# mikael-jorda/sai2-primitives-perso

Measured on AMD Instinct MI355X. Metric: control-ticks/sec (node), 65k batched 7-DOF Panda, 2-task hierarchy, higher is better.
Workload: dtype f64

## Files before the change

### sai2-primitives-perso_amd/csrc/sai2b_fast.hpp

```cpp
#pragma once
#include "sai2b_device.hpp"

namespace sai2b {

template <int n, class Mat>
DI void chol(const Mat& A, real* L, real* dinv) {
	UNROLL for (int j = 0; j < n; j++) {
		real s = A[j * n + j];
		UNROLL for (int k = 0; k < j; k++) s = fma(-L[j * n + k], L[j * n + k], s);
		real r = rsqrt(s);
		dinv[j] = r;
		L[j * n + j] = s * r;
		UNROLL for (int i = j + 1; i < n; i++) {
			real t = A[i * n + j];
			UNROLL for (int k = 0; k < j; k++) t = fma(-L[i * n + k], L[j * n + k], t);
			L[i * n + j] = t * r;
		}
	}
}
template <int n>
DI void solve_lower(const real* L, const real* dinv, real* x) {
	UNROLL for (int i = 0; i < n; i++) {
		real t = x[i];
		UNROLL for (int k = 0; k < i; k++) t = fma(-L[i * n + k], x[k], t);
		x[i] = t * dinv[i];
	}
}
template <int n>
DI void solve_lower_t(const real* L, const real* dinv, real* x) {
	UNROLL for (int i = n - 1; i >= 0; i--) {
		real t = x[i];
		UNROLL for (int k = i + 1; k < n; k++) t = fma(-L[k * n + i], x[k], t);
		x[i] = t * dinv[i];
	}
}

DI bool certify_nonsingular(const real* J, real s_abs_tol, real s_max) {
	real G[36];
	mm_nt_sym<6, N>(J, J, G);
	return certify_gram<6>(G, nullptr, s_abs_tol * s_abs_tol, s_max * s_max);
}

struct JtEarly {
	real f[N], ddq[N], integ[N];
};
template <class Rows>
DI void fast_jt_early(const DevTask& t1, const RobotCtx& rc, const Rows& r, JtEarly& e) {
	UNROLL for (int i = 0; i < N; i++) {
		const real qd = r.law_goal(i), dqd = r.law_goal(N + i);
		e.ddq[i] = r.law_goal(2 * N + i);
		const real integ = fma(rc.q[i] - qd, t1.dt, r.state(i));
		e.integ[i] = integ;
		if (t1.use_vsat) {
			const real kvi = gain_pinv(t1.kv[i]);
			real dv = -t1.kp[i] * kvi * (rc.q[i] - qd) - t1.ki[i] * kvi * integ;
			dv = fmin(fmax(dv, -t1.vsat[i]), t1.vsat[i]);
			e.f[i] = -t1.kv[i] * (rc.dq[i] - dv);
		} else {
			e.f[i] = -t1.kp[i] * (rc.q[i] - qd) - t1.kv[i] * (rc.dq[i] - dqd) - t1.ki[i] * integ;
		}
	}
}

#define SAI2B_PHASE() do { __builtin_amdgcn_sched_barrier(0); asm volatile("; SAI2B_PHASE_MARK"); __builtin_amdgcn_sched_barrier(0); } while (0)
#if defined(__HIP_DEVICE_COMPILE__)
#define SAI2B_CHAIN_PHASE() SAI2B_PHASE()
#endif
}
#include "sai2b_chain.h"
namespace sai2b {

template <int FAST, bool PAY = false>
struct StageLayout {
	static constexpr bool JT_STAGED = FAST == 2 && PAY, PARKED = FAST == 2 && !PAY;
	static constexpr int DQ = 0, JG = N, JS = JG + (JT_STAGED ? 3 * N : 0), MG = JS + (JT_STAGED ? N : 0);
	static constexpr int MS = MG + 24, PLD = MS + 6, ROWS = PLD + (PAY ? PAYLOAD_ROWS : 0);
	static constexpr int PAIRS = (ROWS + 1) / 2;
	static constexpr int IROW = 2 * PAIRS;
	static constexpr int IMAGE = IROW * 64 + 32;
	static constexpr int MROWS = N * (N + 1) / 2;
	static constexpr int DOUBLES = IMAGE + (PARKED ? (MROWS + N) * 64 : 0);
};

template <int FAST, bool PAY = false>
DI const real* stage_row(const DevParams& P, int k) {
	using S = StageLayout<FAST, PAY>;
	const int B = P.B;
	if (k >= S::ROWS) k = S::ROWS - 1;
	if (k < S::JG) return P.dq + (size_t)(k - S::DQ) * B;
	if (k < S::JS) return P.task[1].law_goals + (size_t)(k - S::JG) * B;
	if (k < S::MG) return P.task[1].state + (size_t)(k - S::JS) * B;
	if (k < S::MS) return P.task[0].law_goals + (size_t)(k - S::MG) * B;
	if constexpr (PAY) {
		if (k >= S::PLD) return P.payload + (size_t)(k - S::PLD) * B;
	}
	return P.task[0].state + (size_t)(k - S::MS) * B;
}

DI void glds(const void* src, real* lds, int bytes) {
	typedef __attribute__((address_space(1))) void gvoid;
	typedef __attribute__((address_space(3))) void lvoid;
	if (bytes == 16)
		__builtin_amdgcn_global_load_lds((gvoid*)src, (lvoid*)lds, 16, 0, 0);
	else
		__builtin_amdgcn_global_load_lds((gvoid*)src, (lvoid*)lds, 4, 0, 0);
}

template <int FAST, bool PAY = false>
DI void stage_issue(const DevParams& P, real* img, int b0) {
	using S = StageLayout<FAST, PAY>;
	const int B = P.B, lane = threadIdx.x;
	if ((B & 1) == 0) {
		const int col = min(b0 + 2 * (lane & 31), B - 2);
		const bool hi = lane >= 32;
		UNROLL for (int i = 0; i < S::PAIRS; i++)
			glds((hi ? stage_row<FAST, PAY>(P, 2 * i + 1) : stage_row<FAST, PAY>(P, 2 * i)) + col, img + 2 * i * 64, 16);
	} else {
		UNROLL for (int h = 0; h < 2; h++) {
			const int col = min(b0 + 32 * h + (lane >> 1), B - 1);
			UNROLL for (int k = 0; k < S::ROWS; k++)
				glds((const int*)(stage_row<FAST, PAY>(P, k) + col) + (lane & 1), img + k * 64 + 32 * h, 4);
		}
	}
	glds(P.task[0].istate + (size_t)IS_NTYPES * B + min(b0 + lane, B - 1), img + S::IROW * 64, 4);
}

struct StagedRows {
	const DevTask& t;
	int B, b;
	const real* lg;
	const real* st;
	int st_rows;
	DI real law_goal(int k) const { return lg[k * 64]; }
	DI real goal(int k) const { return ld(t.goals, k, B, b); }
	DI real sensed(int k) const { return ld(t.sensed, k, B, b); }
	DI real state(int k) const { return k < st_rows ? st[k * 64] : ld(t.state, k, B, b); }
};

struct LdsSym {
	const real* col;
	DI real operator[](int k) const {
		const int i = k / N, j = k % N;
		return col[(i * (i + 1) / 2 + j) * 64];
	}
};

struct JtGiven {
	const JtEarly& e;
	DI void prefetch() {}
	DI void prefetch_q() {}
	DI void project(const real* a, real& af, real& aacc) {
		UNROLL for (int i = 0; i < N; i++) {
			af = fma(a[i], e.f[i], af);
			aacc = fma(a[i], e.ddq[i], aacc);
		}
	}
};
struct JtLate {
	const DevTask& t1;
	int B, b;
	const real* dq;
	const real* qrows;
	real lg[3 * N], s[N], q[N];
	struct Rows {
		const real *lg, *s;
		DI real law_goal(int k) const { return lg[k]; }
		DI real state(int k) const { return s[k]; }
	};
	DI void prefetch() {
		UNROLL for (int k = 0; k < 3 * N; k++) lg[k] = ld(t1.law_goals, k, B, b);
		UNROLL for (int i = 0; i < N; i++) s[i] = ld(t1.state, i, B, b);
	}
	DI void prefetch_q() {
		UNROLL for (int i = 0; i < N; i++) q[i] = ld(qrows, i, B, b);
	}
	DI void project(const real* a, real& af, real& aacc) {
		RobotCtx rc;
		UNROLL for (int i = 0; i < N; i++) {
			asm volatile("" : "+v"(q[i]) : "v"(a[0]));
			rc.q[i] = q[i];
			rc.dq[i] = dq[i * 64];
		}
		JtEarly e;
		fast_jt_early(t1, rc, Rows{lg, s}, e);
		UNROLL for (int i = 0; i < N; i++) st(t1.state, i, B, b, e.integ[i]);
		JtGiven{e}.project(a, af, aacc);
	}
};

template <class Mat>
DI void fast_tick_mft(const DevParams& P, const real* J, const Mat& M, const real* Fu, const real* Ff, real* tau) {
	const DevTask& t0 = P.task[0];

	const bool mft_bie = t0.decoupling == SAI2B_BOUNDED_INERTIA_ESTIMATES;
	const bool mft_full = t0.decoupling == SAI2B_FULL_DYNAMIC_DECOUPLING;
	const bool any_bie = mft_bie;
	const real thr = t0.bie_threshold;
	real LB[N * N], dB[N], z[6];
	UNROLL for (int i = 0; i < 6; i++) z[i] = Fu[i];
	if (any_bie) {
		real MB[N * N];
		UNROLL for (int i = 0; i < N; i++) UNROLL for (int j = 0; j <= i; j++) MB[i * N + j] = M[i * N + j];
		UNROLL for (int i = 0; i < N; i++) MB[i * N + i] = fmax(MB[i * N + i], thr);
		chol<N>(MB, LB, dB);
	}
	if (mft_bie) {
		real YB[N * 6], AB[36], LAB[36], dAB[6];
		UNROLL for (int c = 0; c < 6; c++) {
			real colb[N];
			UNROLL for (int i = 0; i < N; i++) colb[i] = J[c * N + i];
			solve_lower<N>(LB, dB, colb);
			UNROLL for (int i = 0; i < N; i++) YB[i * 6 + c] = colb[i];
		}
		UNROLL for (int i = 0; i < 6; i++) UNROLL for (int j = 0; j <= i; j++) {
			real s = 0;
			UNROLL for (int l = 0; l < N; l++) s = fma(YB[l * 6 + i], YB[l * 6 + j], s);
			AB[i * 6 + j] = s;
			AB[j * 6 + i] = s;
		}
		chol<6>(AB, LAB, dAB);
		solve_lower<6>(LAB, dAB, z);
		solve_lower_t<6>(LAB, dAB, z);
	}
	SAI2B_PHASE();
	real L[N * N], dL[N], Y[N * 6];
	chol<N>(M, L, dL);
	UNROLL for (int c = 0; c < 6; c++) {
		real col[N];
		UNROLL for (int i = 0; i < N; i++) col[i] = J[c * N + i];
		solve_lower<N>(L, dL, col);
		UNROLL for (int i = 0; i < N; i++) Y[i * 6 + c] = col[i];
	}
	SAI2B_PHASE();
	if (mft_full) {
		real A[36], LA[36], dA[6];
		UNROLL for (int i = 0; i < 6; i++) UNROLL for (int j = 0; j <= i; j++) {
			real s = 0;
			UNROLL for (int l = 0; l < N; l++) s = fma(Y[l * 6 + i], Y[l * 6 + j], s);
			A[i * 6 + j] = s;
			A[j * 6 + i] = s;
		}
		chol<6>(A, LA, dA);
		solve_lower<6>(LA, dA, z);
		solve_lower_t<6>(LA, dA, z);
	}
	SAI2B_PHASE();
	UNROLL for (int i = 0; i < 6; i++) z[i] += Ff[i];
	real yz[N], tau_mft[N];
	mv<N, 6>(Y, z, yz);
	UNROLL for (int i = 0; i < N; i++) {
		real s = 0;
		UNROLL for (int k = 0; k <= i; k++) s = fma(L[i * N + k], yz[k], s);
		tau_mft[i] = s;
	}
	UNROLL for (int i = 0; i < N; i++) tau[i] = tau_mft[i];
}

template <bool HAS_JT, class Mat, class JT>
DI void fast_tick(const DevParams& P, const real* J, const Mat& M, const real* Fu, const real* Ff, int B, int b,
				  bool with_comp, JT& jt, real* tau) {
	if constexpr (!HAS_JT) {
		fast_tick_mft(P, J, M, Fu, Ff, tau);
	} else {
		const DevTask &t0 = P.task[0], &t1 = P.task[1];
		const bool jt_bie = t1.decoupling == SAI2B_BOUNDED_INERTIA_ESTIMATES;
		chain::tick2<N>(J, M, Fu, Ff, t0.decoupling == SAI2B_BOUNDED_INERTIA_ESTIMATES,
						t0.decoupling == SAI2B_FULL_DYNAMIC_DECOUPLING, t1.decoupling == SAI2B_FULL_DYNAMIC_DECOUPLING,
						t1.decoupling == SAI2B_IMPEDANCE, jt_bie ? t1.bie_threshold : t0.bie_threshold, with_comp, jt, tau);
	}
}

}
```

### sai2-primitives-perso_amd/csrc/sai2b_fast_body.hpp

```cpp
#pragma once
#include <hip/hip_runtime.h>

#include "sai2b_device.hpp"
#include "sai2b_fast.hpp"
#include "sai2b_baked_panda.h"
#include "sai2b_baked_panda_model.h"

namespace sai2b {

#if SAI2B_N == 7
DI void fk(const PandaBaked&, const real* q, Frames& F) {
	real sn[N], cs[N];
	UNROLL for (int i = 0; i < N; i++) sincos_joint(q[i], &sn[i], &cs[i]);
	panda_fk(sn, cs, F);
}
DI void jacobian(const PandaBaked&, const DevTask& t, const Frames& F, const real* x, real* J) { panda_jacobian(F, t.link, x, J); }
DI void mass_matrix(const PandaBaked&, const Frames& F, real* M, const NoPayload& = NoPayload{}) { panda_mass_matrix(F, M); }
DI void mass_matrix(const PandaBaked&, const Frames& F, real* M, const Payload& pl) {
	PayloadTerms pt;
	payload_terms(pl, F, pt);
	panda_mass_matrix_payload(F, pl.link, pt, M);
}
DI void gravity_vector(const PandaBaked&, const Frames& F, real* g, const NoPayload& = NoPayload{}) { panda_gravity_vector(F, g); }
DI void gravity_vector(const PandaBaked&, const Frames& F, real* g, const Payload& pl) {
	PayloadTerms pt;
	payload_terms(pl, F, pt);
	panda_gravity_vector_payload(F, pl.link, pt, g);
}

template <bool BAKED, class PL>
DI void fast_model(const DevParams& P, const Frames& F, const PL& pl, real* M, real* g) {
	if constexpr (BAKED)
		mass_matrix(PandaBaked{}, F, M, pl);
	else
		mass_matrix(P.model, F, M, pl);
	if (P.gravity_comp) {
		if constexpr (BAKED)
			gravity_vector(PandaBaked{}, F, g, pl);
		else
			gravity_vector(P.model, F, g, pl);
	}
	else {
		UNROLL for (int i = 0; i < N; i++) g[i] = 0;
	}
}

template <bool SELF>
DI bool fast_declined(int* __restrict__ fb_counts, int* __restrict__ fb_list, int parity, bool mine, int b) {
	if constexpr (SELF)
		return !mine;
	else
		return worklist_append(fb_counts, fb_list, parity, mine, b, fb_counts + 4);
}

template <bool BAKED, class PL, bool SELF = false>
DI bool tick_fast1_loads(const DevParams& P, int with_comp, int* __restrict__ fb_counts, int* __restrict__ fb_list, int parity,
						 int b) {
	const int B = P.B;
	RobotCtx rc;
	UNROLL for (int i = 0; i < N; i++) {
		rc.q[i] = ld(P.q, i, B, b);
		rc.dq[i] = ld(P.dq, i, B, b);
	}
	const DevTask& t0 = P.task[0];
	const bool clean = ldi(t0.istate, IS_NTYPES, B, b) == 0;
	JtEarly jt;
	MftIn in0;
	mft_load(t0, B, b, in0);
	SAI2B_PHASE();
	real J[6 * N], M[N * N], g[N], Fu[6], Ff[6];
	{
		Frames F;
		if constexpr (BAKED)
			fk(PandaBaked{}, rc.q, F);
		else
			fk(P.model, rc.q, F);
		real x[3], R[9];
		frame_pose(t0, F, x, R);
		if constexpr (BAKED)
			jacobian(PandaBaked{}, t0, F, x, J);
		else
			jacobian(P.model, t0, F, x, J);
		SAI2B_PHASE();
		mft_law(t0, rc, J, x, R, in0, Fu, Ff);
		SAI2B_PHASE();
		if constexpr (PL::on) {
			PL pl;
			payload_load(P.payload, P.payload_link, B, b, pl);
			fast_model<BAKED>(P, F, pl, M, g);
		} else {
			if constexpr (BAKED)
				mass_matrix(PandaBaked{}, F, M);
			else
				mass_matrix(P.model, F, M);
			if (P.gravity_comp) {
				if constexpr (BAKED)
					gravity_vector(PandaBaked{}, F, g);
				else
					gravity_vector(P.model, F, g);
			}
			else {
				UNROLL for (int i = 0; i < N; i++) g[i] = 0;
			}
		}
	}
	SAI2B_PHASE();
	const bool ok = certify_nonsingular(J, t0.s_abs_tol, t0.s_max);
	const bool mine = ok && clean;
	if (fast_declined<SELF>(fb_counts, fb_list, parity, mine, b)) return true;
	mft_store_integrators(t0, B, b, in0);
	SAI2B_PHASE();
	real tau[N];
	JtGiven none{jt};
	fast_tick<false>(P, J, M, Fu, Ff, B, b, with_comp != 0, none, tau);
	UNROLL for (int i = 0; i < N; i++) st(P.tau, i, B, b, tau[i] + g[i]);
	return false;
}

template <int FAST, bool BAKED, class PL, bool SELF = false>
DI bool tick_fast_body(const DevParams* __restrict__ Pp, int with_comp, int* __restrict__ fb_counts, int* __restrict__ fb_list,
					   int parity, real* img) {
	const DevParams& P = *Pp;
	const int B = P.B;
	const int b0 = blockIdx.x * 64, b = b0 + threadIdx.x;
	using S = StageLayout<FAST, PL::on>;
	RobotCtx rc;
	UNROLL for (int i = 0; i < N; i++) {
		rc.q[i] = ld(P.q, i, B, min(b, B - 1));
		asm volatile("" : "+v"(rc.q[i]));
	}
	SAI2B_PHASE();
	stage_issue<FAST, PL::on>(P, img, b0);
	SAI2B_PHASE();
	if (b >= B) return false;
	const DevTask& t0 = P.task[0];
	const real* col = img + threadIdx.x;
	real J[6 * N], x[3], R[9];
	{
		Frames F;
		if constexpr (BAKED)
			fk(PandaBaked{}, rc.q, F);
		else
			fk(P.model, rc.q, F);
		frame_pose(t0, F, x, R);
		if constexpr (BAKED)
			jacobian(PandaBaked{}, t0, F, x, J);
		else
			jacobian(P.model, t0, F, x, J);
		if constexpr (S::PARKED) {
			SAI2B_PHASE();
			real M[N * N], g[N];
			fast_model<BAKED>(P, F, PL{}, M, g);
			real* park = img + S::IMAGE + threadIdx.x;
			UNROLL for (int i = 0; i < N; i++) UNROLL for (int j = 0; j <= i; j++) park[(i * (i + 1) / 2 + j) * 64] = M[i * N + j];
			UNROLL for (int i = 0; i < N; i++) park[(S::MROWS + i) * 64] = g[i];
		}
	}
	SAI2B_PHASE();
	const bool ok = certify_nonsingular(J, t0.s_abs_tol, t0.s_max);
	SAI2B_PHASE();
	__syncthreads();
	UNROLL for (int i = 0; i < N; i++) {
		rc.dq[i] = col[(S::DQ + i) * 64];
		if constexpr (!S::PARKED) rc.q[i] = ld(P.q, i, B, b);
	}
	const bool clean = ((const int*)(img + S::IROW * 64))[threadIdx.x] == 0;
	MftIn in0;
	mft_load(t0, StagedRows{t0, B, b, col + S::MG * 64, col + S::MS * 64, 6}, in0);
	SAI2B_PHASE();
	real Fu[6], Ff[6];
	mft_law(t0, rc, J, x, R, in0, Fu, Ff);
	SAI2B_PHASE();
	real tau[N];
	if constexpr (S::PARKED) {
		const bool mine = ok && clean;
		if (fast_declined<SELF>(fb_counts, fb_list, parity, mine, b)) return true;
		mft_store_integrators(t0, B, b, in0);
		SAI2B_PHASE();
		const real* park = col + S::IMAGE;
		JtLate jt{P.task[1], B, b, col + S::DQ * 64, P.q};
		fast_tick<FAST == 2>(P, J, LdsSym{park}, Fu, Ff, B, b, with_comp != 0, jt, tau);
		UNROLL for (int i = 0; i < N; i++) st(P.tau, i, B, b, tau[i] + park[(S::MROWS + i) * 64]);
	} else {
		real M[N * N], g[N];
		{
			PL pl;
			if constexpr (PL::on) {
				pl.link = P.payload_link;
				pl.m = col[S::PLD * 64];
				UNROLL for (int k = 0; k < 3; k++) pl.c[k] = col[(S::PLD + 1 + k) * 64];
				UNROLL for (int k = 0; k < 6; k++) pl.I[k] = col[(S::PLD + 4 + k) * 64];
			}
			Frames F;
			if constexpr (BAKED)
				fk(PandaBaked{}, rc.q, F);
			else
				fk(P.model, rc.q, F);
			fast_model<BAKED>(P, F, pl, M, g);
		}
		SAI2B_PHASE();
		const bool mine = ok && clean;
		if (fast_declined<SELF>(fb_counts, fb_list, parity, mine, b)) return true;
		JtEarly e;
		if constexpr (FAST == 2) fast_jt_early(P.task[1], rc, StagedRows{P.task[1], B, b, col + S::JG * 64, col + S::JS * 64, N}, e);
		mft_store_integrators(t0, B, b, in0);
		if (FAST == 2) {
			UNROLL for (int i = 0; i < N; i++) st(P.task[1].state, i, B, b, e.integ[i]);
		}
		SAI2B_PHASE();
		JtGiven jt{e};
		fast_tick<FAST == 2>(P, J, M, Fu, Ff, B, b, with_comp != 0, jt, tau);
		UNROLL for (int i = 0; i < N; i++) st(P.tau, i, B, b, tau[i] + g[i]);
	}
	return false;
}
#endif

}
```

### sai2-primitives-perso_amd/csrc/sai2b_host.cpp

```cpp
#include <hip/hip_runtime.h>

#include <algorithm>
#include <cmath>
#include <cstdio>
#include <cstdlib>
#include <chrono>
#include <cstring>
#include <string>
#include <vector>

#include "sai2b_launch.h"
#include "sai2b_snapshot_layout.h"
#include "sai2b_reset_sampler_layout.h"
#include "sai2b_env_sampler_layout.h"
#include "sai2b_model_host.h"
#include "sai2b_baked_panda.h"

using sai2b::DevModel;
using sai2b::rot_from_rpy;
using sai2b::sym3_from6;
using sai2b::DevParams;
using sai2b::DevTask;
using sai2b::TickCall;
using sai2b::TickForm;
using sai2b::WorkList;
constexpr int N = SAI2B_N;

static thread_local std::string g_error;

extern "C" void sai2b_shared_error_set(const char* msg);

struct sai2b_ctx {
	int dof_tag = N;
	int B = 0, T = 0, device = 0;
	bool introspection = false;
	bool models_fresh = false;
	bool params_dirty = true;
	bool baked_model = false;
	bool blocking_sync = false;
	sai2b::RouteSwitches sw;
	sai2b::TickRoute route;
	WorkList fb, rg, otg, tk;
	int* fb_seen = nullptr;
	hipEvent_t fb_seen_ev = nullptr;
	unsigned long long* fb_report = nullptr;
	bool update_pending = false;
	double* q_pose = nullptr;
	bool q_is_pose = true;
	unsigned goals_dirty = ~0u;
	bool otg_all_idle = false, no_otg_idle_skip = false;
	unsigned long long goals_epoch = 0, otg_obs_epoch = 0;
	int* otg_busy_seen = nullptr;
	hipEvent_t otg_seen_ev = nullptr;
	sai2b::DelayedLook otg_look;
	bool goals_exposed = false;
	sai2b_robot_model model;
	sai2b_task_config cfg[SAI2B_MAX_TASKS];
	DevParams h_params;
	DevParams* d_params = nullptr;
	hipStream_t stream = nullptr;
	hipStream_t caller_stream = nullptr;
	hipEvent_t ev_in = nullptr, ev_out = nullptr;
	double *q = nullptr, *dq = nullptr, *tau = nullptr;
	double* status_buf = nullptr;
// ... 552 lines not shown
	d.otg_jerk = (c.use_internal_otg && c.internal_otg_jerk_limited) ? 1 : 0;
	d.otg_n = c.type == SAI2B_JOINT_TASK ? c.task_dof : 6;
	for (int i = 0; i < sai2b::OTG_MD; i++) {
		if (c.type == SAI2B_JOINT_TASK) {
			d.otg_vmax[i] = i < c.task_dof ? c.otg_max_velocity[i] : 0.0;
			d.otg_amax[i] = i < c.task_dof ? c.otg_max_acceleration[i] : 0.0;
			d.otg_jmax[i] = i < c.task_dof ? c.otg_max_jerk[i] : 0.0;
		} else {
			d.otg_vmax[i] = i < 3 ? c.otg_max_linear_velocity : i < 6 ? c.otg_max_angular_velocity : 0.0;
			d.otg_amax[i] = i < 3 ? c.otg_max_linear_acceleration : i < 6 ? c.otg_max_angular_acceleration : 0.0;
			d.otg_jmax[i] = i < 3 ? c.otg_max_linear_jerk : i < 6 ? c.otg_max_angular_jerk : 0.0;
		}
	}
}

template <class T>
static int dev_alloc(sai2b_ctx* ctx, T** p, size_t count) {
	void* v = nullptr;
	HIP_TRY(ctx, hipMalloc(&v, std::max<size_t>(count, 1) * sizeof(T)));
	HIP_TRY(ctx, hipMemsetAsync(v, 0, std::max<size_t>(count, 1) * sizeof(T), ctx->stream));
	ctx->allocs.push_back(v);
	*p = (T*)v;
	return SAI2B_OK;
}

static int popc_reinit(sai2b_ctx* ctx, int task) {
	DevTask& d = ctx->h_params.task[task];
	const size_t B = ctx->B;
	int rc;
	if (!d.popc_f) {
		if ((rc = dev_alloc(ctx, &d.popc_f, 4 * B))) return rc;
		if ((rc = dev_alloc(ctx, &d.popc_i, 3 * B))) return rc;
		if ((rc = dev_alloc(ctx, &d.popc_q, (size_t)sai2b::POPC_RING * B))) return rc;
		ctx->params_dirty = true;
	}
	std::vector<double> f(4 * B, 0.0);
	std::fill(f.begin() + 3 * B, f.end(), 1.0);
	std::vector<int> iv(3 * B, 0);
	std::fill(iv.begin(), iv.begin() + B, sai2b::POPC_MAX_COUNTER);
	HIP_TRY(ctx, hipMemcpyAsync(d.popc_f, f.data(), f.size() * sizeof(double), hipMemcpyHostToDevice, ctx->stream));
	HIP_TRY(ctx, hipMemcpyAsync(d.popc_i, iv.data(), iv.size() * sizeof(int), hipMemcpyHostToDevice, ctx->stream));
	HIP_TRY(ctx, hipStreamSynchronize(ctx->stream));
	return SAI2B_OK;
}

static int upload_params(sai2b_ctx* ctx) {
	if (!ctx->params_dirty) return SAI2B_OK;
	ctx->h_params.any_bie = 0, ctx->h_params.bie_thr = 0;
	for (int t = 0; t < ctx->h_params.n_tasks; t++)
		if (ctx->h_params.task[t].decoupling == SAI2B_BOUNDED_INERTIA_ESTIMATES) {
			ctx->h_params.any_bie = 1;
			ctx->h_params.bie_thr = ctx->h_params.task[t].bie_threshold;
		}
	HIP_TRY(ctx, hipMemcpyAsync(ctx->d_params, &ctx->h_params, sizeof(DevParams), hipMemcpyHostToDevice, ctx->stream));
	DevParams meas;
	if (ctx->js_on) {
		meas = ctx->h_params;
		meas.q = ctx->js_qm, meas.dq = ctx->js_dqm;
		HIP_TRY(ctx, hipMemcpyAsync(ctx->d_params_meas, &meas, sizeof(DevParams), hipMemcpyHostToDevice, ctx->stream));
	}
	HIP_TRY(ctx, hipStreamSynchronize(ctx->stream));
	ctx->params_dirty = false;
	return SAI2B_OK;
}

static int create_impl(sai2b_ctx* ctx, const sai2b_robot_model* model, const sai2b_task_config* tasks, int n_tasks,
					   int batch, int device) {
	int ndev = 0;
	if (hipGetDeviceCount(&ndev) != hipSuccess || ndev <= 0)
		return set_error(ctx, SAI2B_RUNTIME_ERROR, "sai2b_create: no HIP device available (this library has no CPU path)");
	if (device < 0 || device >= ndev) return set_error(ctx, SAI2B_INVALID_ARGUMENT, "sai2b_create: bad device index");
	HIP_TRY(ctx, hipSetDevice(device));
	HIP_TRY(ctx, hipStreamCreateWithFlags(&ctx->stream, hipStreamNonBlocking));
	HIP_TRY(ctx, hipEventCreateWithFlags(&ctx->ev_in, hipEventDisableTiming));
	HIP_TRY(ctx, hipEventCreateWithFlags(&ctx->ev_out, hipEventDisableTiming));
	ctx->B = batch, ctx->T = n_tasks, ctx->device = device;
	ctx->model = *model;
	ctx->sw = sai2b::route_switches_from_env();
	ctx->route = sai2b::TickRoute(ctx->sw);
	ctx->blocking_sync = sai2b::env_flag("SAI2B_BLOCKING_SYNC");
	ctx->no_otg_idle_skip = sai2b::env_flag("SAI2B_NO_OTG_IDLE_SKIP");
	DevParams& hp = ctx->h_params;
	std::memset(&hp, 0, sizeof(hp));
	hp.B = batch, hp.n_tasks = n_tasks;
	sai2b::host_fill_dev_model(*model, hp.model);
	if constexpr (N == 7) {
		using PB = sai2b::PandaBaked;
		const DevModel& m = hp.model;
		ctx->baked_model = std::memcmp(m.E, PB::E, sizeof(m.E)) == 0 && std::memcmp(m.xyz, PB::xyz, sizeof(m.xyz)) == 0 &&
						   std::memcmp(m.mass, PB::mass, sizeof(m.mass)) == 0 && std::memcmp(m.com, PB::com, sizeof(m.com)) == 0 &&
						   std::memcmp(m.inertia, PB::inertia, sizeof(m.inertia)) == 0 &&
						   std::memcmp(m.gravity, PB::gravity, sizeof(m.gravity)) == 0 &&
						   std::memcmp(m.jtype, PB::jtype, sizeof(m.jtype)) == 0;
		if (sai2b::env_flag("SAI2B_NO_BAKED_MODEL")) ctx->baked_model = false;
	}
	const size_t Bs = (size_t)batch;
	int rc;
	if ((rc = dev_alloc(ctx, &ctx->d_params, 1))) return rc;
	if ((rc = dev_alloc(ctx, &ctx->q, N * Bs))) return rc;
	if ((rc = dev_alloc(ctx, &ctx->dq, N * Bs))) return rc;
	if ((rc = dev_alloc(ctx, &ctx->tau, N * Bs))) return rc;
	hp.q = ctx->q, hp.dq = ctx->dq, hp.tau = ctx->tau;
	if ((rc = dev_alloc(ctx, &ctx->q_pose, (size_t)N * Bs))) return rc;
	if ((rc = dev_alloc(ctx, &ctx->fb.counts, 6))) return rc;
	HIP_TRY(ctx, hipHostMalloc((void**)&ctx->fb_report, 3 * sizeof(unsigned long long), hipHostMallocMapped | hipHostMallocCoherent));
	ctx->fb_report[0] = ctx->fb_report[1] = ctx->fb_report[2] = 0;
	HIP_TRY(ctx, hipHostGetDevicePointer((void**)&ctx->fb.report, ctx->fb_report, 0));
	if ((rc = dev_alloc(ctx, &ctx->fb.list, Bs))) return rc;
	if ((rc = dev_alloc(ctx, &ctx->rg.counts, 2))) return rc;
	if ((rc = dev_alloc(ctx, &ctx->rg.list, Bs))) return rc;
	HIP_TRY(ctx, hipHostMalloc((void**)&ctx->fb_seen, 2 * sizeof(int), hipHostMallocDefault));
// ... 3449 lines not shown
```

### sai2-primitives-perso_amd/csrc/sai2b_params.h

```cpp
#pragma once
#include "../../include/sai2b.h"

namespace sai2b {

#ifndef SAI2B_N
#define SAI2B_N 7
#endif
constexpr int N = SAI2B_N;
static_assert(N >= 1 && N <= SAI2B_MAX_DOF, "SAI2B_N");

struct DevModel {
	double E[N][9];
	double xyz[N][3];
	double mass[N];
	double com[N][3];
	double inertia[N][6];
	double q_lower[N], q_upper[N], effort[N];
	double gravity[3];
	int jtype[N];
};

constexpr int OTG_MD = N > 7 ? N : 7;

struct DevTask {
	int type;
	int decoupling;
	double bie_threshold;
	double dt;
	int k0;
	int full_selection;
	double S[N * N];
	double kp[N], kv[N], ki[N];
	int use_vsat;
	double vsat[N];
	int link;
	double frame_pos[3], frame_rot[9];
	int frame_rigid;
	int full_projection;
	int plain_motion;
	double P[36];
	double PU[36];
	int rank;
	int p_lead;
	int in_frame;
	double kp_pos[3], kv_pos[3], ki_pos[3], kp_ori[3], kv_ori[3], ki_ori[3];
	double kp_f[3], kv_f[3], ki_f[3], kp_m[3], kv_m[3], ki_m[3];
	double kff_f, kff_m, max_f, max_m;
	int cl_force, cl_moment, fdim, mdim;
	int passivity;
	double faxis[3], maxis[3];
	double sig[4][9];
	double lin_vsat, ang_vsat;
	double sensor_rot[9], sensor_pos[3];
// ... 20 lines not shown
	double* popc_f;
	int* popc_i;
	double* popc_q;
	double* dbg_tau;
	double* dbg_N;
	double* dbg_sigma;
	double* dbg_J;
	double* dbg_pose;
	double* dbg_F;
};

constexpr int MFT_GOAL_ROWS = 30;
constexpr int MFT_MOTION_GOAL_ROWS = 24;
constexpr int MFT_GOAL_POS = 0, MFT_GOAL_ROT = 3, MFT_GOAL_LIN_VEL = 12, MFT_GOAL_ANG_VEL = 15, MFT_GOAL_LIN_ACC = 18, MFT_GOAL_ANG_ACC = 21,
			  MFT_GOAL_FORCE = 24, MFT_GOAL_MOMENT = 27;
static_assert(MFT_GOAL_ANG_ACC + 3 == MFT_MOTION_GOAL_ROWS && MFT_MOTION_GOAL_ROWS == 24 && MFT_GOAL_FORCE == MFT_MOTION_GOAL_ROWS &&
				  MFT_GOAL_MOMENT + 3 == MFT_GOAL_ROWS && MFT_GOAL_ROWS == 30,
			  "goal rows of a MotionForceTask");
constexpr int OTG_IN = 0;
constexpr int OTG_CI = 5 * OTG_MD;
constexpr int OTG_OUT = 10 * OTG_MD;
constexpr int OTG_TIME = 13 * OTG_MD, OTG_DURATION = OTG_TIME + 1, OTG_GOAL_REACHED = OTG_TIME + 2, OTG_RESULT = OTG_TIME + 3,
			  OTG_TARGET_SET = OTG_TIME + 4, OTG_CI_INIT = OTG_TIME + 5, OTG_CI_EPOCH = OTG_TIME + 6, OTG_CONSTRUCTED = OTG_TIME + 7;
constexpr int OTG_TRAJ = OTG_TIME + 8;
constexpr int OTG_TRAJ_STRIDE = 13;
constexpr int OTG3_BRAKE = 0, OTG3_TSUM = 11, OTG3_J = 18, OTG3_A = 25, OTG3_V = 33, OTG3_P = 41, OTG3_STRIDE = 49;
constexpr int OTG_CART = OTG_TRAJ + OTG_MD * OTG_TRAJ_STRIDE;
constexpr int OTG_CART_REF = OTG_CART, OTG_CART_GOAL_R = OTG_CART + 9, OTG_CART_GOAL_W = OTG_CART + 18;
constexpr int OTG_IN_SYNC = OTG_CART + 21;
constexpr int OTG_ACTIVE = OTG_CART + 22;
constexpr int OTG_ROWS = OTG_CART + 23;
static_assert(N > 7 || (OTG_TRAJ == 99 && OTG_CART == 190 && OTG_IN_SYNC == 211), "row layout of the 7-DoF builds");
constexpr int MFT_QPRIOR = 12, MFT_DQPRIOR = 12 + N, MFT_T2DIR = 12 + 2 * N;
constexpr int MFT_STATE_ROWS = 12 + 3 * N;
constexpr int MFT_ISTATE_ROWS = 12;
constexpr int POPC_RING = 1024;
constexpr int POPC_WINDOW = 250, POPC_MAX_COUNTER = 50;
constexpr int IS_NTYPES = 7, IS_COUNT = 8, IS_SIZE = 9, IS_C1 = 10, IS_C2 = 11;

constexpr int PAYLOAD_ROWS = 10;
constexpr int CONTACT_ROWS = 9;
constexpr int CONTACT_STATUS_ROWS = 2 * SAI2B_MAX_CONTACT_POINTS + 6;

enum TickCertBits {
	TICK_CERT_COMP = 1,
	TICK_CERT_NO_INLANE = 2
};
enum TaskCertBits {
	TASK_CERT_TORQUE = 1,
	TASK_CERT_COMMIT = 2,
	TASK_CERT_NO_INLANE = 4
};

struct DevParams {
	int B;
	int n_tasks;
	int gravity_comp;
	int any_bie;
	const double* q;
	const double* dq;
	double* tau;
	double* dbg_M;
	double bie_thr;
	DevModel model;
	DevTask task[SAI2B_MAX_TASKS];
	const double* payload;
	const double* plant_payload;
	int payload_link, plant_payload_link;
	const double* contact;
	double* contact_status;
	int* contact_count;
	int contact_link, contact_n_points, contact_sensor_task, contact_reserved;
	double contact_points[SAI2B_MAX_CONTACT_POINTS][3];
	double contact_v_eps;
};

}
```

Baseline: 3.428 billion.

## Pack fast-path kernel parameters into cache-line-aligned block with scalar-register loads

Adds a FastBlock to DevParams, filled on the host, that groups the pointers, flags and gains used by the fast tick path into 64-byte-aligned groups. The kernel reads these grouped fields and pins them to scalar registers with inline-asm ties, replacing scattered loads from the large DevTask structs and runtime decoupling comparisons with a precomputed flags word. A specialised plain-motion law and a split Jt gain burst are also added. The aim is fewer, burstier scalar parameter loads and less register pressure, at the cost of duplicated parameter state that must stay in sync with the host fill.

```diff
diff --git a/sai2-primitives-perso_amd/csrc/sai2b_fast.hpp b/sai2-primitives-perso_amd/csrc/sai2b_fast.hpp
--- a/sai2-primitives-perso_amd/csrc/sai2b_fast.hpp
+++ b/sai2-primitives-perso_amd/csrc/sai2b_fast.hpp
@@ -44,22 +44,58 @@
 struct JtEarly {
 	real f[N], ddq[N], integ[N];
 };
+template <class T>
+DI void sgpr_tie(T& v) {
+	asm volatile("" : "+s"(v));
+}
+struct JtGains {
+	real dt, kp[N], kv[N], ki[N], vsat[N];
+};
+template <bool VSAT>
+DI void jt_gains_burst(const FastJt& s, JtGains& g) {
+	g.dt = s.dt;
+	UNROLL for (int i = 0; i < N; i++) {
+		g.kp[i] = s.kp[i], g.kv[i] = s.kv[i], g.ki[i] = s.ki[i];
+		if constexpr (VSAT) g.vsat[i] = s.vsat[i];
+	}
+	sgpr_tie(g.dt);
+	UNROLL for (int i = 0; i < N; i++) {
+		sgpr_tie(g.kp[i]), sgpr_tie(g.kv[i]), sgpr_tie(g.ki[i]);
+		if constexpr (VSAT) sgpr_tie(g.vsat[i]);
+	}
+}
 template <class Rows>
-DI void fast_jt_early(const DevTask& t1, const RobotCtx& rc, const Rows& r, JtEarly& e) {
-	UNROLL for (int i = 0; i < N; i++) {
-		const real qd = r.law_goal(i), dqd = r.law_goal(N + i);
-		e.ddq[i] = r.law_goal(2 * N + i);
-		const real integ = fma(rc.q[i] - qd, t1.dt, r.state(i));
-		e.integ[i] = integ;
-		if (t1.use_vsat) {
-			const real kvi = gain_pinv(t1.kv[i]);
-			real dv = -t1.kp[i] * kvi * (rc.q[i] - qd) - t1.ki[i] * kvi * integ;
-			dv = fmin(fmax(dv, -t1.vsat[i]), t1.vsat[i]);
-			e.f[i] = -t1.kv[i] * (rc.dq[i] - dv);
-		} else {
-			e.f[i] = -t1.kp[i] * (rc.q[i] - qd) - t1.kv[i] * (rc.dq[i] - dqd) - t1.ki[i] * integ;
-		}
-	}
+DI void fast_jt_law(const JtGains& g, bool use_vsat, const RobotCtx& rc, const Rows& r, JtEarly& e) {
+	if (use_vsat) {
+		UNROLL for (int i = 0; i < N; i++) {
+			const real qd = r.law_goal(i);
+			e.ddq[i] = r.law_goal(2 * N + i);
+			const real integ = fma(rc.q[i] - qd, g.dt, r.state(i));
+			e.integ[i] = integ;
+			const real kvi = gain_pinv(g.kv[i]);
+			real dv = -g.kp[i] * kvi * (rc.q[i] - qd) - g.ki[i] * kvi * integ;
+			dv = fmin(fmax(dv, -g.vsat[i]), g.vsat[i]);
+			e.f[i] = -g.kv[i] * (rc.dq[i] - dv);
+		}
+	} else {
+		UNROLL for (int i = 0; i < N; i++) {
+			const real qd = r.law_goal(i), dqd = r.law_goal(N + i);
+			e.ddq[i] = r.law_goal(2 * N + i);
+			const real integ = fma(rc.q[i] - qd, g.dt, r.state(i));
+			e.integ[i] = integ;
+			e.f[i] = -g.kp[i] * (rc.q[i] - qd) - g.kv[i] * (rc.dq[i] - dqd) - g.ki[i] * integ;
+		}
+	}
+}
+
+template <class Rows>
+DI void fast_jt_early(const FastJt& t1, bool use_vsat, const RobotCtx& rc, const Rows& r, JtEarly& e) {
+	JtGains g;
+	if (use_vsat)
+		jt_gains_burst<true>(t1, g);
+	else
+		jt_gains_burst<false>(t1, g);
+	fast_jt_law(g, use_vsat, rc, r, e);
 }
 
 #define SAI2B_PHASE() do { __builtin_amdgcn_sched_barrier(0); asm volatile("; SAI2B_PHASE_MARK"); __builtin_amdgcn_sched_barrier(0); } while (0)
@@ -83,18 +119,18 @@
 };
 
 template <int FAST, bool PAY = false>
-DI const real* stage_row(const DevParams& P, int k) {
+DI const real* stage_row(const FastEntry& P, int k) {
 	using S = StageLayout<FAST, PAY>;
 	const int B = P.B;
 	if (k >= S::ROWS) k = S::ROWS - 1;
 	if (k < S::JG) return P.dq + (size_t)(k - S::DQ) * B;
-	if (k < S::JS) return P.task[1].law_goals + (size_t)(k - S::JG) * B;
-	if (k < S::MG) return P.task[1].state + (size_t)(k - S::JS) * B;
-	if (k < S::MS) return P.task[0].law_goals + (size_t)(k - S::MG) * B;
+	if (k < S::JS) return P.law_goals1 + (size_t)(k - S::JG) * B;
+	if (k < S::MG) return P.state1 + (size_t)(k - S::JS) * B;
+	if (k < S::MS) return P.law_goals0 + (size_t)(k - S::MG) * B;
 	if constexpr (PAY) {
 		if (k >= S::PLD) return P.payload + (size_t)(k - S::PLD) * B;
 	}
-	return P.task[0].state + (size_t)(k - S::MS) * B;
+	return P.state0 + (size_t)(k - S::MS) * B;
 }
 
 DI void glds(const void* src, real* lds, int bytes) {
@@ -107,7 +143,7 @@
 }
 
 template <int FAST, bool PAY = false>
-DI void stage_issue(const DevParams& P, real* img, int b0) {
+DI void stage_issue(const FastEntry& P, real* img, int b0) {
 	using S = StageLayout<FAST, PAY>;
 	const int B = P.B, lane = threadIdx.x;
 	if ((B & 1) == 0) {
@@ -122,7 +158,7 @@
 				glds((const int*)(stage_row<FAST, PAY>(P, k) + col) + (lane & 1), img + k * 64 + 32 * h, 4);
 		}
 	}
-	glds(P.task[0].istate + (size_t)IS_NTYPES * B + min(b0 + lane, B - 1), img + S::IROW * 64, 4);
+	glds(P.istate0 + (size_t)IS_NTYPES * B + min(b0 + lane, B - 1), img + S::IROW * 64, 4);
 }
 
 struct StagedRows {
@@ -137,6 +173,83 @@
 	DI real state(int k) const { return k < st_rows ? st[k * 64] : ld(t.state, k, B, b); }
 };
 
+DI void frame_pose(const FastPose& t, const Frames& F, real* x, real* R) {
+	real Rl[9], pl[3];
+	UNROLL for (int k = 0; k < 9; k++) Rl[k] = F.R[N - 1][k];
+	UNROLL for (int k = 0; k < 3; k++) pl[k] = F.p[N - 1][k];
+	UNROLL for (int i = 0; i < N - 1; i++)
+		if (t.link == i) {
+			UNROLL for (int k = 0; k < 9; k++) Rl[k] = F.R[i][k];
+			UNROLL for (int k = 0; k < 3; k++) pl[k] = F.p[i][k];
+		}
+	UNROLL for (int k = 0; k < 3; k++)
+		x[k] = fma(Rl[3 * k], t.frame_pos[0], fma(Rl[3 * k + 1], t.frame_pos[1], fma(Rl[3 * k + 2], t.frame_pos[2], pl[k])));
+	mm<3, 3, 3>(Rl, t.frame_rot, R);
+}
+template <class MD>
+DI void jacobian(const MD& md, const FastPose& t, const Frames& F, const real* x, real* J) {
+	UNROLL for (int i = 0; i < N; i++) {
+		real z[3] = {F.R[i][2], F.R[i][5], F.R[i][8]};
+		real d[3] = {x[0] - F.p[i][0], x[1] - F.p[i][1], x[2] - F.p[i][2]}, v[3];
+		cross3(z, d, v);
+		const bool on = i <= t.link, pris = md.jtype[i] != 0;
+		UNROLL for (int k = 0; k < 3; k++) {
+			J[k * N + i] = on ? (pris ? z[k] : v[k]) : 0.0;
+			J[(3 + k) * N + i] = (on && !pris) ? z[k] : 0.0;
+		}
+	}
+}
+template <class Rows>
+DI void fast_mft_load(int flags, const Rows& r, MftIn& in) {
+	UNROLL for (int k = 0; k < 3; k++) {
+		in.g_pos[k] = r.law_goal(k);
+		in.g_v[k] = r.law_goal(12 + k);
+		in.g_w[k] = r.law_goal(15 + k);
+		in.g_a[k] = r.law_goal(18 + k);
+		in.g_al[k] = r.law_goal(21 + k);
+		in.g_f[k] = in.g_m[k] = in.s_f[k] = in.s_m[k] = 0;
+	}
+	UNROLL for (int k = 0; k < 9; k++) in.g_rot[k] = r.law_goal(3 + k);
+	UNROLL for (int k = 0; k < 6; k++) in.integ[k] = r.state(k);
+	UNROLL for (int k = 6; k < 12; k++) in.integ[k] = 0;
+	if (flags & FB_USES_FORCE) {
+		UNROLL for (int k = 0; k < 3; k++) {
+			in.g_f[k] = r.goal(24 + k);
+			in.g_m[k] = r.goal(27 + k);
+		}
+		if (flags & (FB_CL_FORCE | FB_CL_MOMENT)) {
+			UNROLL for (int k = 0; k < 3; k++) {
+				in.s_f[k] = r.sensed(k);
+				in.s_m[k] = r.sensed(3 + k);
+			}
+		}
+	}
+	if (flags & (FB_CL_FORCE | FB_CL_MOMENT)) {
+		UNROLL for (int k = 6; k < 12; k++) in.integ[k] = r.state(k);
+	}
+}
+DI void fast_mft_store_integrators(int flags, real* state, int B, int b, const MftIn& in) {
+	UNROLL for (int k = 0; k < 6; k++) st(state, k, B, b, in.integ[k]);
+	if (flags & FB_CL_FORCE) {
+		UNROLL for (int k = 6; k < 9; k++) st(state, k, B, b, in.integ[k]);
+	}
+	if (flags & FB_CL_MOMENT) {
+		UNROLL for (int k = 9; k < 12; k++) st(state, k, B, b, in.integ[k]);
+	}
+}
+DI void fast_mft_law_plain(const FastLaw& t, const real* v, const real* w, const real* x, const real* R, MftIn& in, real* Fu, real* Ff) {
+	real oe[3];
+	orientation_error(in.g_rot, R, oe);
+	UNROLL for (int k = 0; k < 3; k++) {
+		const real ex = x[k] - in.g_pos[k];
+		in.integ[k] = fma(ex, t.dt, in.integ[k]);
+		in.integ[3 + k] = fma(oe[k], t.dt, in.integ[3 + k]);
+		Fu[k] = in.g_a[k] - t.kp_pos[k] * ex - t.kv_pos[k] * (v[k] - in.g_v[k]) - t.ki_pos[k] * in.integ[k];
+		Fu[3 + k] = in.g_al[k] - t.kp_ori[k] * oe[k] - t.kv_ori[k] * (w[k] - in.g_w[k]) - t.ki_ori[k] * in.integ[3 + k];
+		Ff[k] = Ff[3 + k] = 0;
+	}
+}
+
 struct LdsSym {
 	const real* col;
 	DI real operator[](int k) const {
@@ -156,23 +269,35 @@
 		}
 	}
 };
+template <bool EARLY>
 struct JtLate {
-	const DevTask& t1;
+	const FastJt& t1;
+	bool use_vsat;
+	const real* law_goals;
+	real* state;
 	int B, b;
 	const real* dq;
 	const real* qrows;
 	real lg[3 * N], s[N], q[N];
+	JtGains g;
 	struct Rows {
 		const real *lg, *s;
 		DI real law_goal(int k) const { return lg[k]; }
 		DI real state(int k) const { return s[k]; }
 	};
 	DI void prefetch() {
-		UNROLL for (int k = 0; k < 3 * N; k++) lg[k] = ld(t1.law_goals, k, B, b);
-		UNROLL for (int i = 0; i < N; i++) s[i] = ld(t1.state, i, B, b);
+		UNROLL for (int k = 0; k < 3 * N; k++) lg[k] = ld(law_goals, k, B, b);
+		UNROLL for (int i = 0; i < N; i++) s[i] = ld(state, i, B, b);
 	}
 	DI void prefetch_q() {
 		UNROLL for (int i = 0; i < N; i++) q[i] = ld(qrows, i, B, b);
+		if constexpr (EARLY) gains();
+	}
+	DI void gains() {
+		if (use_vsat)
+			jt_gains_burst<true>(t1, g);
+		else
+			jt_gains_burst<false>(t1, g);
 	}
 	DI void project(const real* a, real& af, real& aacc) {
 		RobotCtx rc;
@@ -182,8 +307,11 @@
 			rc.dq[i] = dq[i * 64];
 		}
 		JtEarly e;
-		fast_jt_early(t1, rc, Rows{lg, s}, e);
-		UNROLL for (int i = 0; i < N; i++) st(t1.state, i, B, b, e.integ[i]);
+		asm volatile("; SAI2B_MARK jt_law_begin");
+		if constexpr (!EARLY) gains();
+		fast_jt_law(g, use_vsat, rc, Rows{lg, s}, e);
+		asm volatile("; SAI2B_MARK jt_law_end");
+		UNROLL for (int i = 0; i < N; i++) st(state, i, B, b, e.integ[i]);
 		JtGiven{e}.project(a, af, aacc);
 	}
 };
@@ -256,18 +384,20 @@
 	UNROLL for (int i = 0; i < N; i++) tau[i] = tau_mft[i];
 }
 
+template <class Mat, class JT>
+DI void fast_tick2(int flags, const FastChain& c, const real* J, const Mat& M, const real* Fu, const real* Ff, bool with_comp, JT& jt,
+				   real* tau) {
+	chain::tick2<N>(J, M, Fu, Ff, (flags & FB_MFT_BIE) != 0, (flags & FB_MFT_FULL) != 0, (flags & FB_JT_FULL) != 0,
+					(flags & FB_JT_IMP) != 0, c.bie_threshold, with_comp, jt, tau);
+}
 template <bool HAS_JT, class Mat, class JT>
 DI void fast_tick(const DevParams& P, const real* J, const Mat& M, const real* Fu, const real* Ff, int B, int b,
 				  bool with_comp, JT& jt, real* tau) {
 	if constexpr (!HAS_JT) {
 		fast_tick_mft(P, J, M, Fu, Ff, tau);
 	} else {
-		const DevTask &t0 = P.task[0], &t1 = P.task[1];
-		const bool jt_bie = t1.decoupling == SAI2B_BOUNDED_INERTIA_ESTIMATES;
-		chain::tick2<N>(J, M, Fu, Ff, t0.decoupling == SAI2B_BOUNDED_INERTIA_ESTIMATES,
-						t0.decoupling == SAI2B_FULL_DYNAMIC_DECOUPLING, t1.decoupling == SAI2B_FULL_DYNAMIC_DECOUPLING,
-						t1.decoupling == SAI2B_IMPEDANCE, jt_bie ? t1.bie_threshold : t0.bie_threshold, with_comp, jt, tau);
-	}
-}
-
-}
+		fast_tick2(P.fast.entry.flags, P.fast.chain, J, M, Fu, Ff, with_comp, jt, tau);
+	}
+}
+
+}
diff --git a/sai2-primitives-perso_amd/csrc/sai2b_fast_block.h b/sai2-primitives-perso_amd/csrc/sai2b_fast_block.h
--- /dev/null
+++ b/sai2-primitives-perso_amd/csrc/sai2b_fast_block.h
@@ -0,0 +1,41 @@
+#pragma once
+#include <cstring>
+
+#include "sai2b_params.h"
+
+namespace sai2b {
+
+inline void fast_block_fill(DevParams& P) {
+	const DevTask &t0 = P.task[0], &t1 = P.task[1];
+	FastBlock& f = P.fast;
+	std::memset(&f, 0, sizeof(f));
+	FastEntry& e = f.entry;
+	e.B = P.B;
+	e.flags = (P.gravity_comp ? FB_GRAVITY_COMP : 0) | (t0.plain_motion ? FB_PLAIN_MOTION : 0) |
+			  ((t0.fdim | t0.mdim) != 0 ? FB_USES_FORCE : 0) | (t0.cl_force ? FB_CL_FORCE : 0) | (t0.cl_moment ? FB_CL_MOMENT : 0) |
+			  (t0.use_vsat ? FB_MFT_VSAT : 0) | (t1.use_vsat ? FB_JT_VSAT : 0) |
+			  (t0.decoupling == SAI2B_BOUNDED_INERTIA_ESTIMATES ? FB_MFT_BIE : 0) |
+			  (t0.decoupling == SAI2B_FULL_DYNAMIC_DECOUPLING ? FB_MFT_FULL : 0) |
+			  (t1.decoupling == SAI2B_BOUNDED_INERTIA_ESTIMATES ? FB_JT_BIE : 0) |
+			  (t1.decoupling == SAI2B_FULL_DYNAMIC_DECOUPLING ? FB_JT_FULL : 0) | (t1.decoupling == SAI2B_IMPEDANCE ? FB_JT_IMP : 0);
+	e.q = e.q_again = P.q, e.dq = P.dq, e.tau = P.tau;
+	e.law_goals0 = t0.law_goals, e.state0 = e.state0_again = t0.state, e.istate0 = t0.istate;
+	e.law_goals1 = t1.law_goals, e.state1 = t1.state;
+	e.payload = P.payload, e.payload_link = P.payload_link;
+	FastPose& p = f.pose;
+	std::memcpy(p.frame_pos, t0.frame_pos, sizeof(p.frame_pos));
+	std::memcpy(p.frame_rot, t0.frame_rot, sizeof(p.frame_rot));
+	p.s_abs_tol = t0.s_abs_tol, p.s_max = t0.s_max, p.link = t0.link;
+	FastLaw& l = f.law;
+	l.dt = t0.dt;
+	for (int k = 0; k < 3; k++) {
+		l.kp_pos[k] = t0.kp_pos[k], l.kv_pos[k] = t0.kv_pos[k], l.ki_pos[k] = t0.ki_pos[k];
+		l.kp_ori[k] = t0.kp_ori[k], l.kv_ori[k] = t0.kv_ori[k], l.ki_ori[k] = t0.ki_ori[k];
+	}
+	f.chain.bie_threshold = t1.decoupling == SAI2B_BOUNDED_INERTIA_ESTIMATES ? t1.bie_threshold : t0.bie_threshold;
+	FastJt& j = f.jt;
+	j.dt = t1.dt, j.use_vsat = t1.use_vsat;
+	for (int i = 0; i < N; i++) j.kp[i] = t1.kp[i], j.kv[i] = t1.kv[i], j.ki[i] = t1.ki[i], j.vsat[i] = t1.vsat[i];
+}
+
+}
diff --git a/sai2-primitives-perso_amd/csrc/sai2b_fast_body.hpp b/sai2-primitives-perso_amd/csrc/sai2b_fast_body.hpp
--- a/sai2-primitives-perso_amd/csrc/sai2b_fast_body.hpp
+++ b/sai2-primitives-perso_amd/csrc/sai2b_fast_body.hpp
@@ -15,6 +15,7 @@
 	panda_fk(sn, cs, F);
 }
 DI void jacobian(const PandaBaked&, const DevTask& t, const Frames& F, const real* x, real* J) { panda_jacobian(F, t.link, x, J); }
+DI void jacobian(const PandaBaked&, const FastPose& t, const Frames& F, const real* x, real* J) { panda_jacobian(F, t.link, x, J); }
 DI void mass_matrix(const PandaBaked&, const Frames& F, real* M, const NoPayload& = NoPayload{}) { panda_mass_matrix(F, M); }
 DI void mass_matrix(const PandaBaked&, const Frames& F, real* M, const Payload& pl) {
 	PayloadTerms pt;
@@ -35,6 +36,22 @@
 	else
 		mass_matrix(P.model, F, M, pl);
 	if (P.gravity_comp) {
+		if constexpr (BAKED)
+			gravity_vector(PandaBaked{}, F, g, pl);
+		else
+			gravity_vector(P.model, F, g, pl);
+	}
+	else {
+		UNROLL for (int i = 0; i < N; i++) g[i] = 0;
+	}
+}
+template <bool BAKED, class PL>
+DI void fast_model(const DevParams& P, bool gravity_comp, const Frames& F, const PL& pl, real* M, real* g) {
+	if constexpr (BAKED)
+		mass_matrix(PandaBaked{}, F, M, pl);
+	else
+		mass_matrix(P.model, F, M, pl);
+	if (gravity_comp) {
 		if constexpr (BAKED)
 			gravity_vector(PandaBaked{}, F, g, pl);
 		else
@@ -121,72 +138,99 @@
 DI bool tick_fast_body(const DevParams* __restrict__ Pp, int with_comp, int* __restrict__ fb_counts, int* __restrict__ fb_list,
 					   int parity, real* img) {
 	const DevParams& P = *Pp;
-	const int B = P.B;
+	const FastBlock& fb = P.fast;
+	FastEntry e = fb.entry;
+	sgpr_tie(e.B), sgpr_tie(e.q), sgpr_tie(e.dq), sgpr_tie(e.law_goals0), sgpr_tie(e.state0), sgpr_tie(e.istate0);
+	if constexpr (PL::on) sgpr_tie(e.payload), sgpr_tie(e.law_goals1), sgpr_tie(e.state1);
+	const int B = e.B;
 	const int b0 = blockIdx.x * 64, b = b0 + threadIdx.x;
 	using S = StageLayout<FAST, PL::on>;
 	RobotCtx rc;
-	UNROLL for (int i = 0; i < N; i++) {
-		rc.q[i] = ld(P.q, i, B, min(b, B - 1));
-		asm volatile("" : "+v"(rc.q[i]));
-	}
-	SAI2B_PHASE();
-	stage_issue<FAST, PL::on>(P, img, b0);
+	UNROLL for (int i = 0; i < N; i++) rc.q[i] = ld(e.q, i, B, min(b, B - 1));
+	UNROLL for (int i = 0; i < N; i++) asm volatile("" : "+v"(rc.q[i]));
+	SAI2B_PHASE();
+	stage_issue<FAST, PL::on>(e, img, b0);
 	SAI2B_PHASE();
 	if (b >= B) return false;
 	const DevTask& t0 = P.task[0];
 	const real* col = img + threadIdx.x;
 	real J[6 * N], x[3], R[9];
+	real s_abs_tol, s_max;
 	{
 		Frames F;
-		if constexpr (BAKED)
+		if constexpr (BAKED) {
+			FastPose pose = fb.pose;
 			fk(PandaBaked{}, rc.q, F);
-		else
+			UNROLL for (int k = 0; k < 3; k++) sgpr_tie(pose.frame_pos[k]);
+			UNROLL for (int k = 0; k < 9; k++) sgpr_tie(pose.frame_rot[k]);
+			sgpr_tie(pose.link), sgpr_tie(pose.s_abs_tol), sgpr_tie(pose.s_max);
+			s_abs_tol = pose.s_abs_tol, s_max = pose.s_max;
+			frame_pose(pose, F, x, R);
+			jacobian(PandaBaked{}, pose, F, x, J);
+		} else {
 			fk(P.model, rc.q, F);
-		frame_pose(t0, F, x, R);
-		if constexpr (BAKED)
-			jacobian(PandaBaked{}, t0, F, x, J);
-		else
-			jacobian(P.model, t0, F, x, J);
+			frame_pose(fb.pose, F, x, R);
+			jacobian(P.model, fb.pose, F, x, J);
+		}
 		if constexpr (S::PARKED) {
 			SAI2B_PHASE();
 			real M[N * N], g[N];
-			fast_model<BAKED>(P, F, PL{}, M, g);
+			fast_model<BAKED>(P, BAKED ? (fb.entry.flags & FB_GRAVITY_COMP) != 0 : P.gravity_comp != 0, F, PL{}, M, g);
 			real* park = img + S::IMAGE + threadIdx.x;
 			UNROLL for (int i = 0; i < N; i++) UNROLL for (int j = 0; j <= i; j++) park[(i * (i + 1) / 2 + j) * 64] = M[i * N + j];
 			UNROLL for (int i = 0; i < N; i++) park[(S::MROWS + i) * 64] = g[i];
 		}
 	}
 	SAI2B_PHASE();
-	const bool ok = certify_nonsingular(J, t0.s_abs_tol, t0.s_max);
-	SAI2B_PHASE();
+	if constexpr (!BAKED) s_abs_tol = fb.pose.s_abs_tol, s_max = fb.pose.s_max;
+	const bool ok = certify_nonsingular(J, s_abs_tol, s_max);
+	SAI2B_PHASE();
+	int flags = fb.entry.flags, Bp = fb.entry.B;
+	FastLaw law = fb.law;
 	__syncthreads();
+	sgpr_tie(flags), sgpr_tie(Bp);
 	UNROLL for (int i = 0; i < N; i++) {
 		rc.dq[i] = col[(S::DQ + i) * 64];
-		if constexpr (!S::PARKED) rc.q[i] = ld(P.q, i, B, b);
+		if constexpr (!S::PARKED) rc.q[i] = ld(e.q, i, Bp, b);
 	}
 	const bool clean = ((const int*)(img + S::IROW * 64))[threadIdx.x] == 0;
 	MftIn in0;
-	mft_load(t0, StagedRows{t0, B, b, col + S::MG * 64, col + S::MS * 64, 6}, in0);
+	fast_mft_load(flags, StagedRows{t0, Bp, b, col + S::MG * 64, col + S::MS * 64, 6}, in0);
 	SAI2B_PHASE();
 	real Fu[6], Ff[6];
-	mft_law(t0, rc, J, x, R, in0, Fu, Ff);
+	real v[3], w[3];
+	mv<3, N>(J, rc.dq, v);
+	mv<3, N>(J + 3 * N, rc.dq, w);
+	if (flags & FB_PLAIN_MOTION) {
+		sgpr_tie(law.dt);
+		UNROLL for (int k = 0; k < 3; k++) {
+			sgpr_tie(law.kp_pos[k]), sgpr_tie(law.kv_pos[k]), sgpr_tie(law.ki_pos[k]);
+			sgpr_tie(law.kp_ori[k]), sgpr_tie(law.kv_ori[k]), sgpr_tie(law.ki_ori[k]);
+		}
+		fast_mft_law_plain(law, v, w, x, R, in0, Fu, Ff);
+	} else {
+		mft_law_vw(t0, v, w, x, R, in0, Fu, Ff);
+	}
+	e.tau = fb.entry.tau, e.law_goals1 = fb.entry.law_goals1, e.state1 = fb.entry.state1;
+	e.q_again = fb.entry.q_again, e.state0_again = fb.entry.state0_again;
 	SAI2B_PHASE();
 	real tau[N];
 	if constexpr (S::PARKED) {
 		const bool mine = ok && clean;
 		if (fast_declined<SELF>(fb_counts, fb_list, parity, mine, b)) return true;
-		mft_store_integrators(t0, B, b, in0);
+		sgpr_tie(e.tau), sgpr_tie(e.law_goals1), sgpr_tie(e.state1), sgpr_tie(e.q_again), sgpr_tie(e.state0_again);
+		fast_mft_store_integrators(flags, e.state0_again, Bp, b, in0);
 		SAI2B_PHASE();
 		const real* park = col + S::IMAGE;
-		JtLate jt{P.task[1], B, b, col + S::DQ * 64, P.q};
-		fast_tick<FAST == 2>(P, J, LdsSym{park}, Fu, Ff, B, b, with_comp != 0, jt, tau);
-		UNROLL for (int i = 0; i < N; i++) st(P.tau, i, B, b, tau[i] + park[(S::MROWS + i) * 64]);
+		JtLate<BAKED> jt{fb.jt, (flags & FB_JT_VSAT) != 0, e.law_goals1, e.state1, Bp, b, col + S::DQ * 64, e.q_again};
+		fast_tick2(flags, fb.chain, J, LdsSym{park}, Fu, Ff, with_comp != 0, jt, tau);
+		UNROLL for (int i = 0; i < N; i++) st(e.tau, i, Bp, b, tau[i] + park[(S::MROWS + i) * 64]);
 	} else {
 		real M[N * N], g[N];
 		{
 			PL pl;
 			if constexpr (PL::on) {
-				pl.link = P.payload_link;
+				pl.link = fb.entry.payload_link;
 				pl.m = col[S::PLD * 64];
 				UNROLL for (int k = 0; k < 3; k++) pl.c[k] = col[(S::PLD + 1 + k) * 64];
 				UNROLL for (int k = 0; k < 6; k++) pl.I[k] = col[(S::PLD + 4 + k) * 64];
@@ -196,21 +240,26 @@
 				fk(PandaBaked{}, rc.q, F);
 			else
 				fk(P.model, rc.q, F);
-			fast_model<BAKED>(P, F, pl, M, g);
+			fast_model<BAKED>(P, (flags & FB_GRAVITY_COMP) != 0, F, pl, M, g);
 		}
 		SAI2B_PHASE();
 		const bool mine = ok && clean;
 		if (fast_declined<SELF>(fb_counts, fb_list, parity, mine, b)) return true;
-		JtEarly e;
-		if constexpr (FAST == 2) fast_jt_early(P.task[1], rc, StagedRows{P.task[1], B, b, col + S::JG * 64, col + S::JS * 64, N}, e);
-		mft_store_integrators(t0, B, b, in0);
+		sgpr_tie(e.tau), sgpr_tie(e.state1), sgpr_tie(e.state0_again);
+		JtEarly je;
+		if constexpr (FAST == 2)
+			fast_jt_early(fb.jt, (flags & FB_JT_VSAT) != 0, rc, StagedRows{P.task[1], Bp, b, col + S::JG * 64, col + S::JS * 64, N}, je);
+		fast_mft_store_integrators(flags, e.state0_again, Bp, b, in0);
 		if (FAST == 2) {
-			UNROLL for (int i = 0; i < N; i++) st(P.task[1].state, i, B, b, e.integ[i]);
-		}
-		SAI2B_PHASE();
-		JtGiven jt{e};
-		fast_tick<FAST == 2>(P, J, M, Fu, Ff, B, b, with_comp != 0, jt, tau);
-		UNROLL for (int i = 0; i < N; i++) st(P.tau, i, B, b, tau[i] + g[i]);
+			UNROLL for (int i = 0; i < N; i++) st(e.state1, i, Bp, b, je.integ[i]);
+		}
+		SAI2B_PHASE();
+		JtGiven jt{je};
+		if constexpr (FAST == 2)
+			fast_tick2(flags, fb.chain, J, M, Fu, Ff, with_comp != 0, jt, tau);
+		else
+			fast_tick<false>(P, J, M, Fu, Ff, Bp, b, with_comp != 0, jt, tau);
+		UNROLL for (int i = 0; i < N; i++) st(e.tau, i, Bp, b, tau[i] + g[i]);
 	}
 	return false;
 }
diff --git a/sai2-primitives-perso_amd/csrc/sai2b_host.cpp b/sai2-primitives-perso_amd/csrc/sai2b_host.cpp
--- a/sai2-primitives-perso_amd/csrc/sai2b_host.cpp
+++ b/sai2-primitives-perso_amd/csrc/sai2b_host.cpp
@@ -10,6 +10,7 @@
 #include <vector>
 
 #include "sai2b_launch.h"
+#include "sai2b_fast_block.h"
 #include "sai2b_snapshot_layout.h"
 #include "sai2b_reset_sampler_layout.h"
 #include "sai2b_env_sampler_layout.h"
@@ -668,11 +669,13 @@
 			ctx->h_params.any_bie = 1;
 			ctx->h_params.bie_thr = ctx->h_params.task[t].bie_threshold;
 		}
+	sai2b::fast_block_fill(ctx->h_params);
 	HIP_TRY(ctx, hipMemcpyAsync(ctx->d_params, &ctx->h_params, sizeof(DevParams), hipMemcpyHostToDevice, ctx->stream));
 	DevParams meas;
 	if (ctx->js_on) {
 		meas = ctx->h_params;
 		meas.q = ctx->js_qm, meas.dq = ctx->js_dqm;
+		sai2b::fast_block_fill(meas);
 		HIP_TRY(ctx, hipMemcpyAsync(ctx->d_params_meas, &meas, sizeof(DevParams), hipMemcpyHostToDevice, ctx->stream));
 	}
 	HIP_TRY(ctx, hipStreamSynchronize(ctx->stream));
diff --git a/sai2-primitives-perso_amd/csrc/sai2b_params.h b/sai2-primitives-perso_amd/csrc/sai2b_params.h
--- a/sai2-primitives-perso_amd/csrc/sai2b_params.h
+++ b/sai2-primitives-perso_amd/csrc/sai2b_params.h
@@ -1,4 +1,6 @@
 #pragma once
+#include <cstddef>
+
 #include "../../include/sai2b.h"
 
 namespace sai2b {
@@ -125,6 +127,63 @@
 	TASK_CERT_NO_INLANE = 4
 };
 
+enum FastFlags {
+	FB_GRAVITY_COMP = 1 << 0,
+	FB_PLAIN_MOTION = 1 << 1,
+	FB_USES_FORCE = 1 << 2,
+	FB_CL_FORCE = 1 << 3,
+	FB_CL_MOMENT = 1 << 4,
+	FB_MFT_VSAT = 1 << 5,
+	FB_JT_VSAT = 1 << 6,
+	FB_MFT_BIE = 1 << 7,
+	FB_MFT_FULL = 1 << 8,
+	FB_JT_BIE = 1 << 9,
+	FB_JT_FULL = 1 << 10,
+	FB_JT_IMP = 1 << 11
+};
+struct alignas(64) FastEntry {
+	int B;
+	int flags;
+	const double* q;
+	const double* dq;
+	const double* law_goals0;
+	double* state0;
+	const int* istate0;
+	const double* payload;
+	int payload_link, reserved;
+	double* tau;
+	const double* law_goals1;
+	double* state1;
+	const double* q_again;
+	double* state0_again;
+};
+static_assert(offsetof(FastEntry, tau) == 64, "the entry group is two lines");
+struct alignas(64) FastPose {
+	double frame_pos[3], frame_rot[9];
+	double s_abs_tol, s_max;
+	int link, reserved;
+};
+struct alignas(64) FastLaw {
+	double dt;
+	double kp_pos[3], kv_pos[3], ki_pos[3], kp_ori[3], kv_ori[3], ki_ori[3];
+};
+struct alignas(64) FastChain {
+	double bie_threshold;
+};
+struct alignas(64) FastJt {
+	double dt;
+	double kp[N], kv[N], ki[N];
+	double vsat[N];
+	int use_vsat, reserved;
+};
+struct alignas(64) FastBlock {
+	FastEntry entry;
+	FastPose pose;
+	FastLaw law;
+	FastChain chain;
+	FastJt jt;
+};
+
 struct DevParams {
 	int B;
 	int n_tasks;
@@ -146,6 +205,10 @@
 	int contact_link, contact_n_points, contact_sensor_task, contact_reserved;
 	double contact_points[SAI2B_MAX_CONTACT_POINTS][3];
 	double contact_v_eps;
-};
+	FastBlock fast;
+};
+static_assert(offsetof(DevParams, fast) % 64 == 0 && offsetof(FastBlock, pose) % 64 == 0 && offsetof(FastBlock, law) % 64 == 0 &&
+				  offsetof(FastBlock, chain) % 64 == 0 && offsetof(FastBlock, jt) % 64 == 0,
+			  "every group of the FastBlock starts on a 64-byte line");
 
 }
```

Result: faster. 3.830 billion (median of 6 runs) (+11.7%).
